# tum-vision/scenedino

Hardware: AMD Instinct MI355X
Metric: rendered rays/sec, KITTI-360 192x640x64-sample frustum (higher is better)
Workload: dtype bf16

## Files before the change

### include/sdhip.h

```cpp
#ifndef SDHIP_H
#define SDHIP_H

#include <stdint.h>

#define SD_CAM_WORDS 36
#include <stddef.h>

#ifdef __cplusplus
extern "C" {
#endif

enum sd_dtype { SD_F32 = 0, SD_BF16 = 1, SD_F16 = 2 };

const char *sd_last_error(void);

int sd_abi_version(void);

int sd_field_dtype(int dtype);

int32_t sd_reserve_cus(int32_t n);

int sd_spin(int32_t nblocks, float us, void *stream);

int sd_gen_rays(const float *poses_c2w, const float *Ks, const float *frame_ids,
// ... 81 lines not shown
    int64_t ld_depth, ld_dino, ld_rgb;
    int32_t grid_dtype;
    int32_t pad1;
} sd_render_args;

int sd_render_fused(const sd_render_args *args, const sd_mlp *mlp, void *stream);


int sd_project_grid(const float *grid_nchw, int64_t B, int64_t Hf, int64_t Wf,
                    const sd_mlp *mlp, void *out, void *stream);

int sd_project_grid_nhwc(const float *grid_nhwc, int64_t B, int64_t Hf, int64_t Wf,
                         const sd_mlp *mlp, void *out, void *stream);

int sd_project_grid_nhwc_inputs(const float *grid_nhwc, int64_t B, int64_t Hf, int64_t Wf,
                                const sd_mlp *mlp, void *out, const sd_frame_args *frame,
                                void *stream);

typedef struct sd_head {
    const void *w_pe;
    const void *w_sig;
    const void *w_out;
    const float *b_dino;
    float b_sigma;
    int32_t D;
    int32_t dtype;
} sd_head;

int sd_render_proj(const sd_render_args *args, const sd_head *head, void *stream);

int64_t sd_render_proj_work_bytes(int64_t R, int32_t D);

int32_t sd_render_tile_cap(int32_t bytes);

typedef struct sd_field_args {
    const float *xyz; int64_t B; int64_t P;
    const void *grid; int32_t Hf, Wf;
    const float *cam_f;
    const float *img; int32_t nv, Hc, Wc;
    const float *cam_c;
    float *sigma;
    float *dino;
    float *rgb;
    float *invalid;
    uint8_t *invalid_f;
    int32_t dino_dtype;
    int32_t grid_dtype;
    const int32_t *tile_order;
} sd_field_args;

int sd_field_query(const sd_field_args *args, const sd_mlp *mlp, void *stream);

int sd_composite(const float *z, const float *sigma, const float *feat, int64_t F,
                 const float *rgb, int64_t Cc, int64_t R, int32_t K, int32_t hard_alpha_cap,
                 float *weights, float *alphas, float *depth, float *feat_out, float *rgb_out,
                 void *stream);


int sd_field_gather(const float *xyz, int64_t B, int64_t P, const float *grid_nhwc,
                    int32_t C, int32_t Hf, int32_t Wf, const float *cam_f,
                    const float *img, int32_t nv, int32_t Hc, int32_t Wc,
                    const float *cam_c, void *x_out, int32_t x_dtype ,
                    uint8_t *invalid_f, float *rgb, float *invalid, void *stream);

int sd_field_gather_bwd(const float *xyz, int64_t B, int64_t P, const void *dx,
                        int32_t dx_dtype , int64_t ldx, int32_t C, int32_t Hf,
// ... 304 lines not shown
```

### scenedino_amd/_lib.py

```python
from __future__ import annotations

import ctypes
import os

import torch

_HERE = os.path.dirname(os.path.abspath(__file__))
LIB_PATH = os.environ.get("SDHIP_LIB") or os.path.join(_HERE, "libsdhip.so")
ABI_VERSION = 12
CAM_WORDS = 36

SD_F32 = 0
SD_BF16 = 1
SD_F16 = 2
TORCH_DTYPE = {SD_F32: torch.float32, SD_BF16: torch.bfloat16, SD_F16: torch.float16}
SD_OF_TORCH = {v: k for k, v in TORCH_DTYPE.items()}
FIELD_DTYPE = {SD_F32: SD_F32, SD_BF16: SD_F16, SD_F16: SD_F16}

_vp = ctypes.c_void_p
_i64 = ctypes.c_int64
_i32 = ctypes.c_int32


class SdMlp(ctypes.Structure):
# ... 170 lines not shown
 SD_EPI_NCHW) = range(8)

SIGNATURES = {
    "sd_last_error": [],
    "sd_abi_version": [],
    "sd_field_dtype": [ctypes.c_int],
    "sd_reserve_cus": [ctypes.c_int32],
    "sd_spin": [ctypes.c_int32, ctypes.c_float, _vp],
    "sd_ln_gemm": [ctypes.POINTER(SdGemmArgs), _vp, _vp, _vp, ctypes.c_float, _vp],
    "sd_gen_rays": [_vp, _vp, _vp, _i64, _i64, _i64, ctypes.c_float, ctypes.c_float, _vp, _vp],
    "sd_sample_z": [_vp, _i64, _i64, _i64, ctypes.c_int, _vp, ctypes.c_uint64, ctypes.c_uint64,
                    _vp, _vp],
    "sd_patch_rays": [ctypes.POINTER(SdPatchArgs), _vp],
    "sd_pack_grid": [_vp, _i64, _i64, _i64, _i64, ctypes.c_int, _vp, _vp],
    "sd_pack_image": [_vp, _i64, _i64, _i64, _vp, _vp],
    "sd_cam_records": [_vp, _i64, _vp, _i64, _i64, _vp, _vp],
    "sd_frame_inputs": [_vp, _i64, _i64, _i64, _vp, _vp, _i64, _vp, _i64, _i64, _vp, _vp],
    "sd_render_fused": [ctypes.POINTER(SdRenderArgs), ctypes.POINTER(SdMlp), _vp],
    "sd_field_query": [ctypes.POINTER(SdFieldArgs), ctypes.POINTER(SdMlp), _vp],
    "sd_field_gather": [_vp, _i64, _i64, _vp, _i32, _i32, _i32, _vp, _vp, _i32, _i32, _i32, _vp,
                        _vp, _i32, _vp, _vp, _vp, _vp],
    "sd_field_gather_bwd": [_vp, _i64, _i64, _vp, _i32, _i64, _i32, _i32, _i32, _vp, _vp, _vp],
    "sd_unpack_grid": [_vp, _i64, _i64, _i64, _i64, _vp, _vp],
    "sd_composite_bwd": [_vp, _vp, _vp, _i64, _vp, _i64, _i64, _i32, _i32, _vp, _vp, _vp, _vp,
                         _vp, _vp, _vp, _vp, _vp],
    "sd_project_grid": [_vp, _i64, _i64, _i64, ctypes.POINTER(SdMlp), _vp, _vp],
    "sd_project_grid_nhwc": [_vp, _i64, _i64, _i64, ctypes.POINTER(SdMlp), _vp, _vp],
    "sd_project_grid_nhwc_inputs": [_vp, _i64, _i64, _i64, ctypes.POINTER(SdMlp), _vp,
                                    ctypes.POINTER(SdFrameArgs), _vp],
    "sd_cast_grid": [_vp, _i64, ctypes.c_int, _vp, _vp],
    "sd_render_proj": [ctypes.POINTER(SdRenderArgs), ctypes.POINTER(SdHead), _vp],
    "sd_render_proj_work_bytes": [_i64, _i32],
    "sd_render_tile_cap": [_i32],
    "sd_composite": [_vp, _vp, _vp, _i64, _vp, _i64, _i64, _i32, _i32, _vp, _vp, _vp, _vp, _vp,
                     _vp],
    "sd_voxel_points": [ctypes.POINTER(ctypes.c_double), ctypes.c_double, _i64, _i64, _i64,
                        ctypes.POINTER(ctypes.c_double), _vp, _vp],
    "sd_grow3": [_vp, _i64, _i64, _i64, _vp, _vp],
    "sd_seg_query": [_vp, _i32, _i64, ctypes.POINTER(SdSegHead), _vp, ctypes.c_float, _vp, _vp,
                     _vp, _vp],
    "sd_voxel_fov": [ctypes.POINTER(ctypes.c_double), ctypes.c_double, _i64, _i64, _i64,
                     ctypes.POINTER(ctypes.c_double), ctypes.POINTER(ctypes.c_double), _i32, _i32,
                     _vp, _vp],
    "sd_ssc_confusion": [_vp, _vp, _vp, _vp, _i64, _i64, _i64, ctypes.POINTER(SdSscArgs), _vp,
                         _vp],
    "sd_mlp_train_fwd": [ctypes.POINTER(SdMlpTrainArgs), _vp],
    "sd_mlp_train_bwd": [ctypes.POINTER(SdMlpTrainArgs), _vp],
    "sd_wgrad": [ctypes.POINTER(SdWgradArgs), _vp],
    "sd_mlp_train_wgrad": [ctypes.POINTER(SdMlpWgradArgs), _vp],
    "sd_mlp_train_wgrad_work": [_i32],
    "sd_salience_fwd": [ctypes.POINTER(SdSalienceArgs), _vp],
    "sd_salience_bwd": [ctypes.POINTER(SdSalienceArgs), _vp],
    "sd_gemm": [ctypes.POINTER(SdGemmArgs), _vp],
    "sd_gemm_resid_ln": [ctypes.POINTER(SdGemmArgs), _vp, _vp, ctypes.c_float, _vp, _vp, _vp],
    "sd_attention": [_vp, _vp, _vp, _i32, _i32, _i32, _i32, _i32, ctypes.c_float, _vp, _vp],
    "sd_vit_mlp": [_vp, _vp, _i64, _i32, _i32, _vp, _vp, ctypes.c_float, _vp, _vp, _vp, _vp, _vp,
                   _vp],
    "sd_layernorm": [_vp, _i64, _i32, _vp, _vp, ctypes.c_float, _vp, _i32, _vp],
    "sd_patchify": [_vp, _i32, _i32, _i32, _i32, _i32, ctypes.POINTER(ctypes.c_float),
                    ctypes.POINTER(ctypes.c_float), _vp, _vp, _vp, _vp, _i32, _vp],
    "sd_tokens_to_grid": [_vp, _i32, _i32, _i32, _i32, _i32, _i32, _i32, _vp, _vp],
    "sd_tokens_to_nhwc": [_vp, _i32, _i32, _i32, _i32, _i32, _i32, _vp, _vp],
    "sd_layernorm_nhwc": [_vp, _i32, _i32, _i32, _vp, _vp, ctypes.c_float, _i32, _i32, _i32, _vp, _vp],
    "sd_upsample2x": [_vp, _i32, _i32, _i32, _i32, _vp, _vp],
    "sd_conv_wgrad_parts": [ctypes.POINTER(SdConvWgradArgs)],
    "sd_conv_wgrad_work": [ctypes.POINTER(SdConvWgradArgs)],
# ... 259 lines not shown
                               ptr(out), stream_of(out)), "sd_project_grid")
    return out


def project_grid_inputs(grid, mlp: SdMlp, dtype, img_nchw, poses_w2c, Ks, exact_grid: bool = False):
    if not channels_last(grid):
        img, cam = frame_inputs(img_nchw, poses_w2c, Ks)
        return project_grid(grid, mlp, dtype, exact_grid), img, cam
    lib = load()
    mlp = _with_flags(mlp, exact_grid)
    B, C, H, W = grid.shape
    N, c3, Hc, Wc = img_nchw.shape
    assert c3 == 3, "colour images must have 3 channels"
    w, k, n, sw, sk = _cam_operands(poses_w2c, Ks)
    out = torch.empty(B, H, W, 128, device=grid.device, dtype=TORCH_DTYPE[FIELD_DTYPE[dtype]])
    img = torch.empty(N, Hc, Wc, 4, device=img_nchw.device, dtype=torch.float32)
    cam = torch.empty(*poses_w2c.shape[:-2], CAM_WORDS, device=w.device, dtype=torch.float32)
    fa = SdFrameArgs(img_nchw=ptr(_req(img_nchw, "images")), N=N, H=Hc, W=Wc, out_nhwc4=ptr(img),
                     w2c=ptr(w), s_w=sw, Ks=ptr(k), s_k=sk, n=n, out_cam=ptr(cam))
    _check(lib.sd_project_grid_nhwc_inputs(ptr(_req(grid.permute(0, 2, 3, 1), "grid")), B, H, W,
                                           ctypes.byref(mlp), ptr(out), ctypes.byref(fa),
                                           stream_of(out)), "sd_project_grid_nhwc_inputs")
    return out, img, cam


def render_proj_work_bytes(R: int, D: int) -> int:
    return int(load().sd_render_proj_work_bytes(R, D))


def render_tile_cap(nbytes: int) -> int:
    return int(load().sd_render_tile_cap(int(nbytes)))


def render_proj(args: SdRenderArgs, head: SdHead, ref_tensor):
    lib = load()
    _check(lib.sd_render_proj(ctypes.byref(args), ctypes.byref(head), stream_of(ref_tensor)),
           "sd_render_proj")


def field_query(args: SdFieldArgs, mlp: SdMlp, ref_tensor):
    lib = load()
    _check(lib.sd_field_query(ctypes.byref(args), ctypes.byref(mlp), stream_of(ref_tensor)),
           "sd_field_query")


def voxel_fov(origin, voxel_size, dims, T, cam_k, img_w, img_h, device):
    lib = load()
    nx, ny, nz = (int(d) for d in dims)
    o = (ctypes.c_double * 3)(*[float(v) for v in origin])
    Tm = torch.as_tensor(T, dtype=torch.float64).reshape(-1, 4)[:3].flatten().tolist()
    t = (ctypes.c_double * 12)(*Tm)
    km = (ctypes.c_double * 9)(*torch.as_tensor(cam_k, dtype=torch.float64)
                               .reshape(3, 3).flatten().tolist())
    out = torch.empty(nx * ny * nz, device=device, dtype=torch.uint8)
    _check(lib.sd_voxel_fov(o, float(voxel_size), nx, ny, nz, t, km, int(img_w), int(img_h),
                            ptr(out), stream_of(out)), "sd_voxel_fov")
    return out


def ssc_confusion(pred, sigma, target, fov, args: SdSscArgs, conf):
    lib = load()
    nx, ny, nz = (int(d) for d in pred.shape)
    _check(lib.sd_ssc_confusion(ptr(pred), ptr(sigma), ptr(target), ptr(fov), nx, ny, nz,
                                ctypes.byref(args), ptr(conf), stream_of(conf)),
           "sd_ssc_confusion")

# ... 538 lines not shown
```

### scenedino_amd/csrc/sdhip_tile.hip

```cpp
#include "sdhip_render.h"
#include <stdlib.h>

#ifndef ST_NW_SMALLK
#define ST_NW_SMALLK 8
#endif
#define ST_TEX 288
#define ST_TEXQ 18
#define ST_MAXP 2
#define ST_MAXKW 8

#ifndef ST_PROF
#define ST_PROF 0
#endif
#if ST_PROF
__device__ unsigned long long st_prof[32];
#define ST_T(i)                                                  \
    {                                                            \
        const uint64_t _t = __builtin_amdgcn_s_memtime();        \
        pacc[i] += (uint32_t)(_t - tlast);                       \
        tlast = _t;                                              \
    }
extern "C" int sd_tile_prof(unsigned long long *out, int reset) {
    if (hipMemcpyFromSymbol(out, HIP_SYMBOL(st_prof), sizeof(st_prof)) != hipSuccess) return -2;
    if (reset) {
        unsigned long long z[32] = {0};
        if (hipMemcpyToSymbol(HIP_SYMBOL(st_prof), z, sizeof(z)) != hipSuccess) return -2;
    }
    return 0;
}
#elif defined(ST_MARK) && ST_MARK
#define ST_T(i) asm volatile(";@T " #i)
#else
#define ST_T(i)
#endif
#ifndef ST_MARK
#define ST_MARK 0
#endif
#if ST_MARK
#define ST_M(i) asm volatile(";@M " #i)
#define ST_MV(i, x) asm volatile(";@M " #i : "+v"(x))
#else
// ... 12 lines not shown
#endif
#ifndef ST_SAME_CAM
#define ST_SAME_CAM 1
#endif
#ifndef ST_FASTPROJ
#define ST_FASTPROJ 1
#endif
#if ST_FASTPROJ
#define ST_GEO sd_point_geo_fast
#define ST_CTAPS sd_color_taps_fast
#else
#define ST_GEO sd_point_geo<true>
#define ST_CTAPS sd_color_taps
#endif

struct st_args {
    sd_render_args a;
    sd_head m;
    int32_t *ovf;
    int32_t ovf_cap;
    int32_t ngroups;
    int32_t tile_bytes;
};

#define ST_L_BOX 0
#define ST_HS_ROW 272
__host__ __device__ constexpr int st_l_hs(int nw) { return ST_L_BOX + 2 * nw * 32; }
__host__ __device__ constexpr int st_l_ws(int nw, int rpw) { return st_l_hs(nw) + nw * rpw * ST_HS_ROW; }
__host__ __device__ constexpr int st_l_ray(int nw, int rpw) { return st_l_ws(nw, rpw) + 16 * 4; }
__host__ __device__ constexpr int st_l_rec(int nw, int rpw) { return st_l_ray(nw, rpw) + nw * 2 * 32 * rpw; }
static_assert(st_l_rec(8, 1) % 16 == 0 && st_l_rec(12, 1) % 16 == 0 && st_l_rec(8, 2) % 16 == 0,
              "record area alignment");

__host__ __device__ constexpr int st_rec_bytes(int nw, int kw) { return nw * 2 * kw * 40; }

#define ST_BFLY(NOP, out, a, b, RA, RB, MA, MB)                                               \
    asm volatile(NOP "v_add_f32_dpp %0, %1, %1 row_ror:" #RA " row_mask:0xf bank_mask:" #MA "\n\t" \
                 "v_add_f32_dpp %0, %2, %2 row_ror:" #RB " row_mask:0xf bank_mask:" #MB      \
                 : "=&v"(out) : "v"(a), "v"(b))

__device__ __forceinline__ uint32_t st_min2(uint32_t a, uint32_t b) {
    typedef __attribute__((ext_vector_type(2))) unsigned short u16x2;
    return __builtin_bit_cast(uint32_t, __builtin_elementwise_min(__builtin_bit_cast(u16x2, a),
                                                                  __builtin_bit_cast(u16x2, b)));
}
__device__ __forceinline__ uint32_t st_max2(uint32_t a, uint32_t b) {
    typedef __attribute__((ext_vector_type(2))) unsigned short u16x2;
    return __builtin_bit_cast(uint32_t, __builtin_elementwise_max(__builtin_bit_cast(u16x2, a),
                                                                  __builtin_bit_cast(u16x2, b)));
}
template <bool MAX>
__device__ __forceinline__ uint32_t st_row_red2(uint32_t v) {
#define ST_RSTEP(ctrl)                                                                        \
    {                                                                                         \
        const uint32_t o = (uint32_t)__builtin_amdgcn_mov_dpp((int)v, (ctrl), 0xf, 0xf, false); \
        v = MAX ? st_max2(v, o) : st_min2(v, o);                                              \
    }
    ST_RSTEP(0xB1)
    ST_RSTEP(0x4E)
    ST_RSTEP(0x141)
    ST_RSTEP(0x140)
#undef ST_RSTEP
    return v;
}
template <bool MAX>
__device__ __forceinline__ uint32_t st_rows2(uint32_t v, int r0, int r1) {
    uint32_t acc = (uint32_t)__builtin_amdgcn_readlane((int)v, 16 * r0);
// ... 27 lines not shown
#define ST_EARLY_HW ST_WAIT_EARLY
#endif
#ifndef ST_PRIO
#define ST_PRIO 0
#endif
#ifndef ST_EARLY_FETCH
#define ST_EARLY_FETCH 1
#endif
typedef unsigned u32x4v __attribute__((ext_vector_type(4)));
__device__ __forceinline__ void st_out(float *p, float v) {
    if (ST_WT)
        __hip_atomic_store(p, v, __ATOMIC_RELAXED, __HIP_MEMORY_SCOPE_AGENT);
    else
        *p = v;
}

__device__ __forceinline__ void st_dma4(const void *src, uint32_t lds_addr) {
    lds_addr = __builtin_amdgcn_readfirstlane(lds_addr);
    asm volatile("s_mov_b32 m0, %1\n\ts_nop 0\n\tglobal_load_lds_dword %0, off"
                 :: "v"(src), "s"(lds_addr) : "memory");
}
__device__ __forceinline__ void st_dma_buf16(__amdgpu_buffer_rsrc_t rs, uint32_t voff, uint32_t soff,
                                             uint32_t lds_addr) {
    asm volatile("s_mov_b32 m0, %2\n\ts_nop 0\n\tbuffer_load_dwordx4 %0, %1, %3 offen lds"
                 :: "v"(voff), "s"(rs), "s"(lds_addr), "s"(soff) : "memory");
}
typedef __attribute__((ext_vector_type(4))) short s16x4;

__device__ __forceinline__ uint2 st_tr(uint32_t addr) {
    const s16x4 v = __builtin_amdgcn_ds_read_tr16_b64_v4i16((__attribute__((address_space(3))) s16x4 *)(uintptr_t)addr);
    return __builtin_bit_cast(uint2, v);
}

template <int P, bool ZIN, int NW, int RPW>
__global__ void __launch_bounds__(64 * NW) __attribute__((amdgpu_waves_per_eu(NW / 4)))
k_render_tile(const st_args sa) {
#ifndef ST_HPRE_RPW2
#define ST_HPRE_RPW2 2
#endif
    constexpr int HPRE = (RPW == 2 && ST_HEAD_PRE == 3) ? ST_HPRE_RPW2 : ST_HEAD_PRE;
    constexpr int ST_WAVES = NW;
    constexpr int GR = NW * RPW;
    constexpr int ST_L_HS = st_l_hs(NW), ST_L_WS = st_l_ws(NW, RPW), ST_L_RAY = st_l_ray(NW, RPW),
                  ST_L_REC = st_l_rec(NW, RPW);
    typedef typename RMode<P>::F Tr;
    typedef typename RMode<P>::H Th;
    typedef typename Tr::Frag Frag;
    typedef typename Tr::Frag4 Frag4;
    typedef typename Tr::E E;
    const sd_render_args &a = sa.a;
    const sd_head &m = sa.m;
    extern __shared__ __attribute__((aligned(16))) uint8_t lds[];
#if ST_PROF
    uint32_t pacc[19] = {};
    uint64_t tlast = __builtin_amdgcn_s_memtime();
#endif
    const uint32_t lds0 = (uint32_t)(uintptr_t)(lds_void *)lds;

    const int lane = threadIdx.x & 63, j = lane & 15, g = lane >> 4;
    const int wave = __builtin_amdgcn_readfirstlane(threadIdx.x >> 6);
    const int K = a.K, nsub = K >> 4;
    const int KW = K * RPW, nsubw = KW >> 4;
    const int R = (int)a.R, rps = (int)a.rays_per_sb;
    const int D = m.D, ndt = D >> 4;
    const int Wf = a.Wf, Hf = a.Hf;
    const uint32_t plane_bytes = (uint32_t)Hf * Wf * SD_DH * 2;

    const uint32_t rec_base = ST_L_REC + (uint32_t)wave * 2 * KW * 40;
    auto rq0 = [&](int buf) { return (uint4 *)(lds + rec_base + buf * KW * 40); };
    auto rq1 = [&](int buf) { return (f32x4 *)(lds + rec_base + buf * KW * 40 + KW * 16); };
    auto rqc = [&](int buf) { return (float2 *)(lds + rec_base + buf * KW * 40 + KW * 32); };
    const uint32_t tile0 = ST_L_REC + st_rec_bytes(NW, KW);

    const int NG = sa.ngroups;
    const int nx = (gridDim.x % 8 == 0) ? 8 : 1;
    const int xcd = blockIdx.x % nx, lb = blockIdx.x / nx, nwg = gridDim.x / nx;
    const int glo = (int)((int64_t)NG * xcd / nx), ghi = (int)((int64_t)NG * (xcd + 1) / nx);
    const int gfirst = glo + lb;
    const int nsteps = gfirst < ghi ? (ghi - gfirst + nwg - 1) / nwg : 0;
    int novf = 0;
    int32_t *ovf_list = sa.ovf + gridDim.x + (int64_t)blockIdx.x * sa.ovf_cap;
    if (nsteps == 0) {
        if (threadIdx.x == 0) sa.ovf[blockIdx.x] = 0;
        return;
    }

    const float zstep = (float)(1.0 / (double)K), zend = (float)(1.0 - 1.0 / (double)K);
    const int64_t cplane = (int64_t)a.Hc * a.Wc * 4;

    const int nrw = min(a.ray_dim, 8);
    auto rmap = [&](int ray_, int r) { return RPW == 1 ? ray_ + r : ray_ - RPW * wave + r * NW + wave; };
    auto ray_fetch = [&](int ray, int slot) {
        const int r = lane >> 3, w = lane & 7;
        if (r < RPW && w < nrw && rmap(ray, r) < R)
            st_dma4(a.rays + (int64_t)rmap(ray, r) * a.ray_dim + w,
                    lds0 + ST_L_RAY + (wave * 2 + slot) * 32 * RPW);
    };
    const int rsl = RPW == 1 ? 0 : min(lane / K, RPW - 1);
    auto rsl_p = [&](int p) { return RPW == 1 ? 0 : min((64 * p + lane) / K, RPW - 1); };
    auto kl_p = [&](int p) { return RPW == 1 ? 64 * p + lane : 64 * p + lane - rsl_p(p) * K; };
    const float *rl = nullptr;
    auto load_ray_z = [&](int ray, float zq[2 * ST_MAXP]) {
        float zo[ST_MAXP];
        if (ZIN) {
            if (RPW == 1) {
// ... 116 lines not shown
            q[1] = st_rows2<true>(mx0, 0, 1);
            q[2] = st_rows2<false>(mn0, 2, 3);
            q[3] = st_rows2<true>(mx0, 2, 3);
            q[4] = st_rows2<false>(mn1, 0, 1);
            q[5] = st_rows2<true>(mx1, 0, 1);
            q[6] = st_rows2<false>(mn1, 2, 3);
            q[7] = st_rows2<true>(mx1, 2, 3);
            ST_T(12);
            if (lane == 0) {
                *(uint4 *)bw = uint4{q[0], q[1], q[2], q[3]};
                *(uint4 *)(bw + 16) = uint4{q[4], q[5], q[6], q[7]};
            }
        } else {
            bmin0 = st_wave_min2(bmin0);
            bmax0 = st_wave_max2(bmax0);
            bmin1 = st_wave_min2(bmin1);
            bmax1 = st_wave_max2(bmax1);
            ST_T(12);
            if (lane == 0) *(uint4 *)bw = uint4{bmin0, bmax0, bmin1, bmax1};
        }
    };
    auto ray_col = [&](int ray, int buf) {
        if (rmap(ray, rsl) < R && lane < KW) {
            float col[3];
            sd_color_finish(cpend, col);
            rq0(buf)[lane].w = __builtin_bit_cast(uint32_t, col[0]);
            rqc(buf)[lane] = float2{col[1], col[2]};
        }
    };

    struct Tile {
        int bx0, by0, tw, th, pitch, ok, split;
    };
    const int NPART = (KW == 64 || (RPW == 2 && KW == 128)) ? 4 : 2;
    auto box_union = [&](int slot, int p0, int p1, uint32_t &mn, uint32_t &mx) {
        const uint4 *bx = (const uint4 *)(lds + ST_L_BOX + slot * ST_WAVES * 32);
        mn = 0xffffffffu;
        mx = 0u;
        if (lane < 2 * ST_WAVES) {
            const uint4 v = bx[lane];
            const int pa = 2 * (lane & 1);
            if (pa >= p0 && pa < p1) {
                mn = v.x;
                mx = v.y;
            }
            if (pa + 1 >= p0 && pa + 1 < p1) {
                mn = st_min2(mn, v.z);
                mx = st_max2(mx, v.w);
            }
        }
        static_assert(2 * ST_WAVES <= 16, "box entries in lane row 0");
        mn = st_rows2<false>(st_row_red2<false>(mn), 0, 0);
        mx = st_rows2<true>(st_row_red2<true>(mx), 0, 0);
    };
    auto geom = [&](uint32_t mn, uint32_t mx) {
        Tile t;
        t.bx0 = (int)(mn & 0xffffu);
        t.by0 = (int)(mn >> 16);
        t.tw = (int)(mx & 0xffffu) - t.bx0 + 1;
        t.th = (int)(mx >> 16) - t.by0 + 1;
        t.pitch = t.tw > 0 ? st_pitch(t.tw) : 1;
        t.ok = (mn != 0xffffffffu) && t.tw > 0 && t.th > 0 &&
               t.th * t.pitch * ST_TEX <= sa.tile_bytes && (t.tw * ST_TEXQ + 63) / 64 <= ST_MAXKW * ST_WAVES;
        t.split = 0;
        return t;
    };
    auto dma = [&](const Tile &t, int tb, int sbi) {
// ... 71 lines not shown
            gp[p] = t.pitch;
        }
        const int np = t.split + 1;
#pragma unroll 1
        for (int q = 1; q < np; ++q) {
            uint32_t mn1, mx1;
            box_union(rbuf, q * NPART / np, (q + 1) * NPART / np, mn1, mx1);
            const Tile tq = geom(mn1, mx1);
            const int s0 = q * nsubw / np, s1 = (q + 1) * nsubw / np;
#pragma unroll
            for (int p = 0; p < ST_MAXP; ++p) {
                const int it = (64 * p + lane) >> 4;
                const bool mine = it >= s0 && it < s1;
                gx[p] = mine ? tq.bx0 : gx[p];
                gy[p] = mine ? tq.by0 : gy[p];
                gp[p] = mine ? tq.pitch : gp[p];
            }
        }
        const uint32_t tbase = lds0 + tile0 + (uint32_t)tb * (uint32_t)sa.tile_bytes;
        uint32_t *w = (uint32_t *)rq0(rbuf);
#pragma unroll
        for (int p = 0; p < ST_MAXP; ++p) {
            const int k = 64 * p + lane;
            if (64 * p < KW && k < KW) {
                const uint32_t xy = w[4 * k];
                const int bx0 = gx[p], by0 = gy[p], pch = gp[p];
                const int x0 = (int)(xy & 0x7fffu), y0 = (int)((xy >> 15) & 0x7fffu);
                const uint32_t ad = tbase + (uint32_t)(((y0 - by0) * pch + (x0 - bx0)) * ST_TEX);
                w[4 * k] = ad | (xy & 0xc0000000u);
            }
        }
    };

    typedef typename Th::Frag HFrag;
#ifndef ST_BD_HOIST1
#define ST_BD_HOIST1 0
#endif
    constexpr bool BDH = RPW == 2 || ST_BD_HOIST1;
    f32x4 bdw = {0.f, 0.f, 0.f, 0.f};
    if (BDH && wave < ndt) bdw = *(const f32x4 *)(m.b_dino + 16 * wave + 4 * g);
    auto head_w = [&](int dt, HFrag w[4]) {
        const HFrag *wo = (const HFrag *)m.w_out + (int64_t)dt * 4 * SD_WAVE + lane;
#pragma unroll
        for (int s = 0; s < 4; ++s) w[s] = wo[s * SD_WAVE];
    };
    auto head = [&](int grp, const HFrag w0[4]) {
        if (wave >= ndt) return;
        const int slot = j < GR ? j : 0;
        typename Th::Frag Bh[4];
        const uint8_t *hs = lds + ST_L_HS + slot * ST_HS_ROW;
#pragma unroll
        for (int s = 0; s < 4; ++s) {
            const uint2 lo = *(const uint2 *)(hs + (32 * s + 4 * g) * 2);
            const uint2 hi = *(const uint2 *)(hs + (32 * s + 16 + 4 * g) * 2);
            Bh[s] = __builtin_bit_cast(typename Th::Frag, uint4{lo.x, lo.y, hi.x, hi.y});
        }
        const float ws = *(const float *)(lds + ST_L_WS + slot * 4);
        const int ray = GR * grp + (RPW == 1 ? j : (j % RPW) * NW + j / RPW);
        const bool store = j < GR && ray < R;
        for (int dt = wave; dt < ndt; dt += ST_WAVES) {
            HFrag wl[4];
            if ((HPRE == 1 || HPRE == 3) && dt == wave) {
#pragma unroll
                for (int s = 0; s < 4; ++s) wl[s] = w0[s];
            } else {
                head_w(dt, wl);
// ... 15 lines not shown
                        (uint32_t)(((int64_t)(ray - GR * grp) * a.ld_dino + dim) * 4), 0, 16);
                } else {
                    *(f32x4 *)(a.dino + (int64_t)ray * a.ld_dino + dim) = res;
                }
            }
        }
    };

    const int tq = (lane & 15) >> 2, tp = lane & 3;
    const bool bsel = ((j & 7) >> 1) == g;
    const bool bc0 = bsel && (j >> 3) == 0, bc1 = bsel && (j >> 3) == 1;
    const bool br1 = (j & 1) != 0;
    const f32x4 zero4 = {0.f, 0.f, 0.f, 0.f};
    Frag wpe[8];
    Frag4 wpe1[8];
#pragma unroll
    for (int t = 0; t < 8; ++t) {
        wpe[t] = ((const Frag *)m.w_pe)[t * SD_WAVE + lane];
        wpe1[t] = ((const Frag4 *)((const uint8_t *)m.w_pe + 8 * SD_WAVE * 16))[t * SD_WAVE + lane];
    }
    uint4 wsig_r[4];
#pragma unroll
    for (int s2 = 0; s2 < 4; ++s2) wsig_r[s2] = ((const uint4 *)m.w_sig)[s2 * SD_WAVE + lane];
#if ST_WAIT_FIX
    __builtin_amdgcn_s_waitcnt(0x0F70);
#endif

    int grp = gfirst;
    int ray = GR * grp + RPW * wave;
    int sbi = __builtin_amdgcn_readfirstlane((int)((unsigned)min(GR * grp, R - 1) / (unsigned)rps));
    ray_fetch(ray, 0);
    ray_fetch(GR * (grp + nwg) + RPW * wave, 1);
    asm volatile("s_waitcnt vmcnt(0)" ::: "memory");
    ray_pass(ray, 0, 0);
    ray_col(ray, 0);
    st_barrier_lds();
    Tile cur = stage(0, 0, grp, sbi);
    tap_addrs(0, 0, cur, ray);
    asm volatile("s_waitcnt vmcnt(0)" ::: "memory");
    __syncthreads();

    if (ST_PRIO == 1 && wave >= NW / 2) __builtin_amdgcn_s_setprio(1);
    if (ST_PRIO == 2 && wave < NW / 2) __builtin_amdgcn_s_setprio(1);
    int prev_grp = -1, prev_ok = 0;
    HFrag hwn[4];
#if ST_PROF
#pragma unroll
    for (int i = 0; i < 19; ++i) pacc[i] = 0;
    tlast = __builtin_amdgcn_s_memtime();
#endif
    for (int n = 0; n < nsteps; ++n) {
        const int buf = n & 1;
        const bool has_next = n + 1 < nsteps;
        const int ngrp = grp + nwg;
        const int nray = GR * ngrp + RPW * wave;
        const int nsbi = has_next ? __builtin_amdgcn_readfirstlane((int)((unsigned)min(GR * ngrp, R - 1) / (unsigned)rps)) : 0;
        uint32_t lane_off = (uint32_t)((tq & 1) + (tq >> 1) * cur.pitch) * ST_TEX + 8u * (uint32_t)tp;

        float Tc, dpart, wpart, cpart[3];
#if ST_HC16
        f16x2 hacc16[16];
#else
        f32x4 hacc[8];
#endif
        auto reset = [&]() {
            Tc = 1.f;
            dpart = wpart = cpart[0] = cpart[1] = cpart[2] = 0.f;
#if ST_HC16
#pragma unroll
            for (int i = 0; i < 16; ++i) hacc16[i] = f16x2{(_Float16)0.f, (_Float16)0.f};
#else
#pragma unroll
            for (int t = 0; t < 8; ++t) hacc[t] = zero4;
// ... 85 lines not shown
            cpart[1] += w * st.col[1];
            cpart[2] += w * st.col[2];
            ST_MV(27, cpart[2]);
#if ST_HC16
            const f16x2 ww = __builtin_bit_cast(f16x2, sd_pack2<_Float16>(w, w));
#pragma unroll
            for (int s2 = 0; s2 < 4; ++s2) {
                const uint4 u = __builtin_bit_cast(uint4, st.X[s2]);
                const uint32_t d4[4] = {u.x, u.y, u.z, u.w};
#pragma unroll
                for (int q = 0; q < 4; ++q)
                    hacc16[4 * s2 + q] = __builtin_elementwise_fma(__builtin_bit_cast(f16x2, d4[q]), ww,
                                                                   hacc16[4 * s2 + q]);
            }
#else
            const uint32_t wl = sd_pack2<E>(w, 0.f), wh = sd_pack2<E>(0.f, w);
#pragma unroll
            for (int s2 = 0; s2 < 4; ++s2) {
                const uint4 u = __builtin_bit_cast(uint4, st.X[s2]);
                const uint32_t d4[4] = {u.x, u.y, u.z, u.w};
#pragma unroll
                for (int q = 0; q < 4; ++q) {
                    const int t = 2 * s2 + (q >> 1), r = 2 * (q & 1);
                    hacc[t][r] = Tr::dot2(d4[q], wl, hacc[t][r]);
                    hacc[t][r + 1] = Tr::dot2(d4[q], wh, hacc[t][r + 1]);
                }
            }
#endif
            if (g == 0) *(float2 *)&rq1(buf)[k] = float2{w, st.alpha};
            ST_M(28);
        };

        HFrag hw[4];
        if (HPRE == 1 && prev_ok && wave < ndt) head_w(wave, hw);
        if (HPRE == 2 && prev_ok) head(prev_grp, hw);
        if (HPRE == 3 && prev_ok) head(prev_grp, hwn);
        if (HPRE >= 2) ST_T(1);
        if (has_next) ray_pass(nray, buf ^ 1, buf ^ 1);
        ST_T(0);
        if (HPRE < 2 && prev_ok) head(prev_grp, hw);
        if (HPRE < 2) ST_T(1);
        IState s0;
        if (cur.ok && ray < R) itemA(0, s0);
        ST_T(2);
        if (has_next) ray_col(nray, buf ^ 1);
        ST_T(3);
        st_barrier_lds();
        ST_T(4);
        Tile nxt = {0, 0, 0, 0, 1, 0, 0};
        if (has_next) {
            nxt = stage(buf ^ 1, buf ^ 1, ngrp, nsbi);
            tap_addrs(buf ^ 1, buf ^ 1, nxt, nray);
        }
        if (ST_EARLY_FETCH && n + 2 < nsteps) ray_fetch(GR * (ngrp + nwg) + RPW * wave, buf);
        if (ST_EARLY_HW && HPRE == 3 && cur.ok && wave < ndt) head_w(wave, hwn);
        ST_T(5);
        const int npart = cur.split + 1;
        int qn = 1, bnd = npart > 1 ? nsubw / npart : nsubw;
        auto ray_sums = [&](int r) {
            const float dsum = sd_rowsum16(dpart), wsum = sd_rowsum16(wpart);
            const float c0s = sd_rowsum16(cpart[0]), c1s = sd_rowsum16(cpart[1]),
                        c2s = sd_rowsum16(cpart[2]);
            uint8_t *hs = lds + ST_L_HS + (wave * RPW + r) * ST_HS_ROW;
            {
#if ST_HC16
                float hacc[8][4];
#pragma unroll
                for (int s2 = 0; s2 < 4; ++s2)
#pragma unroll
                    for (int q = 0; q < 4; ++q) {
                        const int t = 2 * s2 + (q >> 1), r = 2 * (q & 1);
                        const uint32_t hb = __builtin_bit_cast(uint32_t, hacc16[4 * s2 + q]);
                        hacc[t][r] = (float)__builtin_bit_cast(_Float16, (uint16_t)(hb & 0xffffu));
                        hacc[t][r + 1] = (float)__builtin_bit_cast(_Float16, (uint16_t)(hb >> 16));
                    }
#endif
                float u[16], v[8];
                asm volatile("s_nop 1" : "+v"(hacc[0][0]), "+v"(hacc[0][1]), "+v"(hacc[0][2]), "+v"(hacc[0][3]),
                             "+v"(hacc[1][0]), "+v"(hacc[1][1]), "+v"(hacc[1][2]), "+v"(hacc[1][3]),
                             "+v"(hacc[2][0]), "+v"(hacc[2][1]), "+v"(hacc[2][2]), "+v"(hacc[2][3]),
                             "+v"(hacc[3][0]), "+v"(hacc[3][1]), "+v"(hacc[3][2]), "+v"(hacc[3][3]));
                asm volatile("s_nop 1" : "+v"(hacc[4][0]), "+v"(hacc[4][1]), "+v"(hacc[4][2]), "+v"(hacc[4][3]),
                             "+v"(hacc[5][0]), "+v"(hacc[5][1]), "+v"(hacc[5][2]), "+v"(hacc[5][3]),
                             "+v"(hacc[6][0]), "+v"(hacc[6][1]), "+v"(hacc[6][2]), "+v"(hacc[6][3]),
                             "+v"(hacc[7][0]), "+v"(hacc[7][1]), "+v"(hacc[7][2]), "+v"(hacc[7][3]));
// ... 48 lines not shown
                if (act) ray_sums(r);
                reset();
            }
        }
        if (ST_WAIT_EARLY) asm volatile("s_waitcnt vmcnt(0)" ::: "memory");
        ST_T(6);
        if (cur.ok && rmap(ray, RPW - 1) < R) ray_sums(RPW - 1);
        if (cur.ok) {
#pragma unroll
            for (int p = 0; p < ST_MAXP; ++p) {
                const int kr = 64 * p + lane;
                const int rr = RPW == 1 ? 0 : min(kr / K, RPW - 1);
                const int k = kr - rr * K;
                if (64 * p < KW && kr < KW && rmap(ray, rr) < R) {
                    const int64_t rk = (int64_t)rmap(ray, rr) * K;
                    const f32x4 q1v = rq1(buf)[kr];
                    const uint4 q0v = rq0(buf)[kr];
                    const uint32_t fl = q0v.x >> 30;
                    if (a.weights) st_out(a.weights + rk + k, q1v[0]);
                    if (a.alphas) st_out(a.alphas + rk + k, q1v[1]);
                    if (a.invalid_f) a.invalid_f[rk + k] = (uint8_t)(fl & 1u);
                    if (a.invalid) st_out(a.invalid + rk + k, fl ? 1.f : 0.f);
                    if (a.rgb_samps) {
                        const float2 cgb = rqc(buf)[kr];
                        float *rsp = a.rgb_samps + (rk + k) * 3;
                        st_out(rsp, __builtin_bit_cast(float, q0v.w));
                        st_out(rsp + 1, cgb.x);
                        st_out(rsp + 2, cgb.y);
                    }
                }
            }
        }
        ST_T(7);
        prev_grp = grp;
        prev_ok = cur.ok;
        grp = ngrp;
        ray = nray;
        sbi = nsbi;
        cur = nxt;
        if (!ST_EARLY_FETCH && n + 2 < nsteps) ray_fetch(GR * (ngrp + nwg) + RPW * wave, buf);
        if (!ST_EARLY_HW && HPRE == 3 && prev_ok && wave < ndt) head_w(wave, hwn);
        if (!ST_WAIT_EARLY) asm volatile("s_waitcnt vmcnt(0)" ::: "memory");
        ST_T(8);
        st_barrier_lds();
        ST_T(9);
    }
    if (threadIdx.x == 0) sa.ovf[blockIdx.x] = novf;
    if (prev_ok) {
        if (HPRE == 1) {
            HFrag hw[4];
            if (wave < ndt) head_w(wave, hw);
            head(prev_grp, hw);
        } else {
            head(prev_grp, hwn);
        }
    }
#if ST_PROF
    if (lane < 19) {
        uint32_t v = 0;
#pragma unroll
        for (int i = 0; i < 19; ++i) v = lane == i ? pacc[i] : v;
        atomicAdd(&st_prof[lane], (unsigned long long)v);
    }
    if (lane == 0) atomicAdd(&st_prof[31], 1ull);
#endif
}

static int sd_check_last(const char *what) {
    hipError_t e = hipGetLastError();
    if (e != hipSuccess) {
        sd_set_error(hipGetErrorString(e));
        (void)what;
        return -2;
    }
    return 0;
}

static int st_nw(int K) { return K <= 64 ? ST_NW_SMALLK : 8; }

static int st_rpw(int K) {
    static const int force = getenv("SDHIP_TILE_RPW") ? atoi(getenv("SDHIP_TILE_RPW")) : 0;
    const int kmax = force == 2 ? 64 : 32;
    return (K <= kmax && force != 1 && st_nw(K) == 8) ? 2 : 1;
}

static int st_lds_fixed(int K) {
    const int nw = st_nw(K), rpw = st_rpw(K);
    return st_l_rec(nw, rpw) + st_rec_bytes(nw, K * rpw);
}

static int st_cap_bytes = 0;
extern "C" int32_t sd_render_tile_cap(int32_t bytes) {
    const int prev = st_cap_bytes;
    st_cap_bytes = bytes > 0 ? bytes : 0;
    return prev;
}

static int st_tile_bytes(int K) {
    const int avail = 160 * 1024 - st_lds_fixed(K);
    const int b = ((avail / 2) / 1024) * 1024;
    return st_cap_bytes ? min(b, (st_cap_bytes / 1024) * 1024) : b;
}

extern "C" int sd_render_tile_ok(const sd_render_args *a, const sd_head *m) {
    return a->nv == 1 && a->K % 16 == 0 && a->K <= 128 &&
           a->rays_per_sb % (st_nw(a->K) * st_rpw(a->K)) == 0 &&
           m->D % 16 == 0 && m->D <= 512 && a->Wf < 32768 && a->Hf < 32768 &&
           st_tile_bytes(a->K) >= 16 * 1024;
}

extern "C" int sd_render_tile_launch(const sd_render_args *a, const sd_head *m, int32_t *ovf,
                                     void *stream) {
    hipStream_t s = (hipStream_t)stream;
    st_args sa;
    sa.a = *a;
    sa.m = *m;
    sa.ovf = ovf;
    const int ncu = sd_num_cus();
    sa.ovf_cap = (int32_t)sd_ovf_cap(a->R, ncu);
    const int nw = st_nw(a->K), rpw = st_rpw(a->K);
    sa.ngroups = (int)((a->R + nw * rpw - 1) / (nw * rpw));
    sa.tile_bytes = st_tile_bytes(a->K);
    const int lds_bytes = st_lds_fixed(a->K) + 2 * sa.tile_bytes;
    auto go = [&](auto kern) {
        sd_lds_attr((const void *)kern, lds_bytes);
        hipLaunchKernelGGL(kern, dim3((unsigned)ncu), dim3(64 * nw), lds_bytes, s, sa);
    };
    const bool zin = a->z != nullptr;
#define ST_GO(NWV, RPWV)                                                                              \
    if (m->dtype == SD_F16) {                                                                         \
        if (zin) go(k_render_tile<SD_F16, true, NWV, RPWV>); else go(k_render_tile<SD_F16, false, NWV, RPWV>); \
    } else {                                                                                          \
        if (zin) go(k_render_tile<SD_BF16, true, NWV, RPWV>); else go(k_render_tile<SD_BF16, false, NWV, RPWV>); \
    }
    if (nw == 8 && rpw == 2) {
        ST_GO(8, 2)
    } else if (nw == 8) {
        ST_GO(8, 1)
    } else {
        ST_GO(ST_NW_SMALLK, 1)
    }
#undef ST_GO
    return sd_check_last("sd_render_proj (tile kernel)");
}
```

Measured before the change: 211.7 million.

## Add late-order tile schedule: box pass first, per-sample geometry after staging

Adds a LATE variant of the tile render kernel. It first computes only a conservative bounding box from a few sample points per ray, stages the feature tile, and then recomputes the full per-sample geometry, tap records and colour after the tile loads are issued, overlapping that work with the loads. Rays whose samples fall outside the predicted box are flagged through LDS and sent to the overflow list. This halves the record buffering in LDS, which leaves room for larger tiles. It is the default for K=64 with RPW=2 and accepts non-divisible rays_per_sb when there is a single superbatch. The trade-off is duplicated geometry work, a coarse box estimate that can send more groups to the overflow path, and a changed meaning for the SDHIP_TILE_RPW env var.

```diff
diff --git a/include/sdhip.h b/include/sdhip.h
--- a/include/sdhip.h
+++ b/include/sdhip.h
@@ -137,6 +137,8 @@
 int64_t sd_render_proj_work_bytes(int64_t R, int32_t D);
 
 int32_t sd_render_tile_cap(int32_t bytes);
+
+int32_t sd_render_tile_order(int32_t order);
 
 typedef struct sd_field_args {
     const float *xyz; int64_t B; int64_t P;
diff --git a/scenedino_amd/_lib.py b/scenedino_amd/_lib.py
--- a/scenedino_amd/_lib.py
+++ b/scenedino_amd/_lib.py
@@ -226,6 +226,7 @@
     "sd_render_proj": [ctypes.POINTER(SdRenderArgs), ctypes.POINTER(SdHead), _vp],
     "sd_render_proj_work_bytes": [_i64, _i32],
     "sd_render_tile_cap": [_i32],
+    "sd_render_tile_order": [_i32],
     "sd_composite": [_vp, _vp, _vp, _i64, _vp, _i64, _i64, _i32, _i32, _vp, _vp, _vp, _vp, _vp,
                      _vp],
     "sd_voxel_points": [ctypes.POINTER(ctypes.c_double), ctypes.c_double, _i64, _i64, _i64,
@@ -551,6 +552,10 @@
     return int(load().sd_render_tile_cap(int(nbytes)))
 
 
+def render_tile_order(order: int) -> int:
+    return int(load().sd_render_tile_order(int(order)))
+
+
 def render_proj(args: SdRenderArgs, head: SdHead, ref_tensor):
     lib = load()
     _check(lib.sd_render_proj(ctypes.byref(args), ctypes.byref(head), stream_of(ref_tensor)),
diff --git a/scenedino_amd/csrc/sdhip_tile.hip b/scenedino_amd/csrc/sdhip_tile.hip
--- a/scenedino_amd/csrc/sdhip_tile.hip
+++ b/scenedino_amd/csrc/sdhip_tile.hip
@@ -7,6 +7,7 @@
 #define ST_TEX 288
 #define ST_TEXQ 18
 #define ST_MAXP 2
+#define ST_BOX_EPS (1.f / 1024.f)
 #define ST_MAXKW 8
 
 #ifndef ST_PROF
@@ -85,7 +86,9 @@
 static_assert(st_l_rec(8, 1) % 16 == 0 && st_l_rec(12, 1) % 16 == 0 && st_l_rec(8, 2) % 16 == 0,
               "record area alignment");
 
-__host__ __device__ constexpr int st_rec_bytes(int nw, int kw) { return nw * 2 * kw * 40; }
+__host__ __device__ constexpr int st_rec_bytes(int nw, int kw, bool late = false) {
+    return late ? nw * kw * 40 + 16 : nw * 2 * kw * 40;
+}
 
 #define ST_BFLY(NOP, out, a, b, RA, RB, MA, MB)                                               \
     asm volatile(NOP "v_add_f32_dpp %0, %1, %1 row_ror:" #RA " row_mask:0xf bank_mask:" #MA "\n\t" \
@@ -179,7 +182,7 @@
     return __builtin_bit_cast(uint2, v);
 }
 
-template <int P, bool ZIN, int NW, int RPW>
+template <int P, bool ZIN, int NW, int RPW, bool LATE = false>
 __global__ void __launch_bounds__(64 * NW) __attribute__((amdgpu_waves_per_eu(NW / 4)))
 k_render_tile(const st_args sa) {
 #ifndef ST_HPRE_RPW2
@@ -206,18 +209,19 @@
 
     const int lane = threadIdx.x & 63, j = lane & 15, g = lane >> 4;
     const int wave = __builtin_amdgcn_readfirstlane(threadIdx.x >> 6);
-    const int K = a.K, nsub = K >> 4;
+    const int K = LATE ? 128 / RPW : a.K, nsub = K >> 4;
     const int KW = K * RPW, nsubw = KW >> 4;
     const int R = (int)a.R, rps = (int)a.rays_per_sb;
     const int D = m.D, ndt = D >> 4;
     const int Wf = a.Wf, Hf = a.Hf;
     const uint32_t plane_bytes = (uint32_t)Hf * Wf * SD_DH * 2;
 
-    const uint32_t rec_base = ST_L_REC + (uint32_t)wave * 2 * KW * 40;
-    auto rq0 = [&](int buf) { return (uint4 *)(lds + rec_base + buf * KW * 40); };
-    auto rq1 = [&](int buf) { return (f32x4 *)(lds + rec_base + buf * KW * 40 + KW * 16); };
-    auto rqc = [&](int buf) { return (float2 *)(lds + rec_base + buf * KW * 40 + KW * 32); };
-    const uint32_t tile0 = ST_L_REC + st_rec_bytes(NW, KW);
+    const uint32_t rec_base = ST_L_REC + (uint32_t)wave * (LATE ? 1 : 2) * KW * 40;
+    auto rq0 = [&](int buf) { return (uint4 *)(lds + rec_base + (LATE ? 0 : buf) * KW * 40); };
+    auto rq1 = [&](int buf) { return (f32x4 *)(lds + rec_base + (LATE ? 0 : buf) * KW * 40 + KW * 16); };
+    auto rqc = [&](int buf) { return (float2 *)(lds + rec_base + (LATE ? 0 : buf) * KW * 40 + KW * 32); };
+    const uint32_t tile0 = ST_L_REC + st_rec_bytes(NW, KW, LATE);
+    const uint32_t flag0 = tile0 - 16;
 
     const int NG = sa.ngroups;
     const int nx = (gridDim.x % 8 == 0) ? 8 : 1;
@@ -400,7 +404,7 @@
     struct Tile {
         int bx0, by0, tw, th, pitch, ok, split;
     };
-    const int NPART = (KW == 64 || (RPW == 2 && KW == 128)) ? 4 : 2;
+    const int NPART = (LATE || KW == 64 || (RPW == 2 && KW == 128)) ? 4 : 2;
     auto box_union = [&](int slot, int p0, int p1, uint32_t &mn, uint32_t &mx) {
         const uint4 *bx = (const uint4 *)(lds + ST_L_BOX + slot * ST_WAVES * 32);
         mn = 0xffffffffu;
@@ -538,6 +542,136 @@
         }
     };
 
+    auto samp_geo = [&](const float *rw, int rmem, int k, int sbi_, float &z0, float &px, float &py,
+                        float &pz) {
+        if (ZIN)
+            z0 = a.z[(int64_t)rmem * K + k];
+        else
+            z0 = sd_z_sample_rng(rw[6], rw[7], K, k,
+                                 sd_uniform(a.z_seed, a.z_offset + (uint64_t)rmem * (uint64_t)K + k), zstep,
+                                 zend, a.z_lindisp);
+        px = rw[0] + z0 * rw[3];
+        py = rw[1] + z0 * rw[4];
+        pz = rw[2] + z0 * rw[5];
+        return ST_GEO((sd_cfloat *)(a.cam_f + sbi_ * SD_CAM_WORDS), px, py, pz, Wf, Hf);
+    };
+    auto box_pass = [&](int ray_, int slot, int sbi_) {
+        const int e = lane & 7;
+        const int kr = 32 * (e >> 1) + ((e & 1) ? 31 : 0);
+        const int r = RPW == 1 ? 0 : kr / K, k = kr - r * K;
+        const int rmem = rmap(ray_, r);
+        uint32_t mn = 0xffffffffu, mx = 0u;
+        if (rmem < R) {
+            const float *rw = (const float *)(lds + ST_L_RAY + (wave * 2 + slot) * 32 * RPW) + 8 * r;
+            float z0, px, py, pz;
+            const PointGeo geo = samp_geo(rw, rmem, k, sbi_, z0, px, py, pz);
+            const float fx = geo.t.w01 + geo.t.w11, fy = geo.t.w10 + geo.t.w11;
+            const int xl = max(geo.t.x0 - (fx < ST_BOX_EPS ? 1 : 0), 0);
+            const int yl = max(geo.t.y0 - (fy < ST_BOX_EPS ? 1 : 0), 0);
+            const int xh = min(geo.t.x0 + (fx > 1.f - ST_BOX_EPS ? 1 : 0), Wf - 1);
+            const int yh = min(geo.t.y0 + (fy > 1.f - ST_BOX_EPS ? 1 : 0), Hf - 1);
+            mn = (uint32_t)xl | ((uint32_t)yl << 16);
+            mx = ((uint32_t)xh | ((uint32_t)yh << 16)) + 0x00010001u;
+        }
+        mn = st_min2(mn, (uint32_t)__builtin_amdgcn_mov_dpp((int)mn, 0xB1, 0xf, 0xf, false));
+        mx = st_max2(mx, (uint32_t)__builtin_amdgcn_mov_dpp((int)mx, 0xB1, 0xf, 0xf, false));
+        uint32_t q[8];
+#pragma unroll
+        for (int i = 0; i < 4; ++i) {
+            q[2 * i] = (uint32_t)__builtin_amdgcn_readlane((int)mn, 2 * i);
+            q[2 * i + 1] = (uint32_t)__builtin_amdgcn_readlane((int)mx, 2 * i);
+        }
+        if (lane == 0) {
+            uint8_t *bw = lds + ST_L_BOX + (slot * ST_WAVES + wave) * 32;
+            *(uint4 *)bw = uint4{q[0], q[1], q[2], q[3]};
+            *(uint4 *)(bw + 16) = uint4{q[4], q[5], q[6], q[7]};
+        }
+    };
+    auto late_pass = [&](int ray_, int slot, int tb, const Tile &t, int sbi_) {
+        if (!t.ok) return;
+        int gx[ST_MAXP], gy[ST_MAXP], gp[ST_MAXP], gw[ST_MAXP], gh[ST_MAXP];
+#pragma unroll
+        for (int p = 0; p < ST_MAXP; ++p) {
+            gx[p] = t.bx0;
+            gy[p] = t.by0;
+            gp[p] = t.pitch;
+            gw[p] = t.tw;
+            gh[p] = t.th;
+        }
+        const int np = t.split + 1;
+#pragma unroll 1
+        for (int q = 1; q < np; ++q) {
+            uint32_t mn1, mx1;
+            box_union(slot, q * NPART / np, (q + 1) * NPART / np, mn1, mx1);
+            const Tile tq = geom(mn1, mx1);
+            const int s0 = q * nsubw / np, s1 = (q + 1) * nsubw / np;
+#pragma unroll
+            for (int p = 0; p < ST_MAXP; ++p) {
+                const int it = (64 * p + lane) >> 4;
+                const bool mine = it >= s0 && it < s1;
+                gx[p] = mine ? tq.bx0 : gx[p];
+                gy[p] = mine ? tq.by0 : gy[p];
+                gp[p] = mine ? tq.pitch : gp[p];
+                gw[p] = mine ? tq.tw : gw[p];
+                gh[p] = mine ? tq.th : gh[p];
+            }
+        }
+        const uint32_t tbase = lds0 + tile0 + (uint32_t)tb * (uint32_t)sa.tile_bytes;
+        const float *rl_ = (const float *)(lds + ST_L_RAY + (wave * 2 + slot) * 32 * RPW);
+        const bool same_cam = ST_SAME_CAM && a.cam_c == a.cam_f && a.Wc == Wf && a.Hc == Hf;
+        uint4 *r0 = rq0(0);
+        f32x4 *r1 = rq1(0);
+        float2 *rc = rqc(0);
+        bool miss = false;
+#pragma unroll
+        for (int p = 0; p < ST_MAXP; ++p) {
+            const int kr = 64 * p + lane;
+            const int r = RPW == 1 ? 0 : kr / K, k = kr - r * K;
+            const int rmem = rmap(ray_, r);
+            if (rmem < R) {
+                float z0, px, py, pz;
+                const PointGeo geo = samp_geo(rl_ + 8 * r, rmem, k, sbi_, z0, px, py, pz);
+                bool ic;
+                Taps tc;
+                if (same_cam) {
+                    tc = geo.t;
+                    ic = geo.inv_f;
+                } else {
+                    tc = ST_CTAPS((sd_cfloat *)(a.cam_c + sbi_ * SD_CAM_WORDS), a.Wc, a.Hc, px, py, pz, ic);
+                }
+                const int dx = geo.t.x0 - gx[p], dy = geo.t.y0 - gy[p];
+                miss |= (uint32_t)dx >= (uint32_t)(gw[p] - 1) || (uint32_t)dy >= (uint32_t)(gh[p] - 1);
+                const uint32_t ad = tbase + (uint32_t)((dy * gp[p] + dx) * ST_TEX);
+                const uint32_t xy = (ad & 0x3fffffffu) | (geo.inv_f ? 1u << 30 : 0u) | (ic ? 1u << 31 : 0u);
+                const uint4 wp = sd_pack_w<SD_F16>(geo.t.w00, geo.t.w01, geo.t.w10, geo.t.w11);
+                r1[kr] = f32x4{geo.v[0], geo.v[1], geo.v[2], z0};
+                if (p == 0) {
+                    sd_color_issue(a.img + (int64_t)sbi_ * cplane, tc, cpend);
+                    r0[kr] = uint4{xy, wp.x, wp.y, 0u};
+                } else {
+                    float col[3];
+                    sd_sample_rgb(a.img + (int64_t)sbi_ * cplane, tc, col);
+                    r0[kr] = uint4{xy, wp.x, wp.y, __builtin_bit_cast(uint32_t, col[0])};
+                    rc[kr] = float2{col[1], col[2]};
+                }
+            }
+        }
+        if (__builtin_amdgcn_ballot_w64(miss) != 0ull && lane == 0)
+            *(volatile uint32_t *)(lds + flag0 + 4 * slot) = 1u;
+    };
+    auto late_check = [&](int slot, Tile &t, int g_) {
+        if (!t.ok) return;
+        const uint32_t f = (uint32_t)__builtin_amdgcn_readfirstlane(
+            (int)*(volatile uint32_t *)(lds + flag0 + 4 * slot));
+        if (!f) return;
+        t.ok = 0;
+        if (wave == 0 && lane == 0) {
+            for (int b = 0; b < GR / SD_LIST_BLK; ++b)
+                ovf_list[novf + b] = g_ * (GR / SD_LIST_BLK) + b;
+        }
+        novf += GR / SD_LIST_BLK;
+    };
+
     typedef typename Th::Frag HFrag;
 #ifndef ST_BD_HOIST1
 #define ST_BD_HOIST1 0
@@ -619,13 +753,26 @@
     ray_fetch(ray, 0);
     ray_fetch(GR * (grp + nwg) + RPW * wave, 1);
     asm volatile("s_waitcnt vmcnt(0)" ::: "memory");
-    ray_pass(ray, 0, 0);
-    ray_col(ray, 0);
-    st_barrier_lds();
-    Tile cur = stage(0, 0, grp, sbi);
-    tap_addrs(0, 0, cur, ray);
-    asm volatile("s_waitcnt vmcnt(0)" ::: "memory");
-    __syncthreads();
+    Tile cur;
+    if constexpr (LATE) {
+        static_assert(HPRE >= 2, "late order: the head runs in front of the box pass");
+        if (threadIdx.x == 0) *(uint2 *)(lds + flag0) = uint2{0u, 0u};
+        box_pass(ray, 0, sbi);
+        st_barrier_lds();
+        cur = stage(0, 0, grp, sbi);
+        late_pass(ray, 0, 0, cur, sbi);
+        asm volatile("s_waitcnt vmcnt(0)" ::: "memory");
+        __syncthreads();
+        late_check(0, cur, grp);
+    } else {
+        ray_pass(ray, 0, 0);
+        ray_col(ray, 0);
+        st_barrier_lds();
+        cur = stage(0, 0, grp, sbi);
+        tap_addrs(0, 0, cur, ray);
+        asm volatile("s_waitcnt vmcnt(0)" ::: "memory");
+        __syncthreads();
+    }
 
     if (ST_PRIO == 1 && wave >= NW / 2) __builtin_amdgcn_s_setprio(1);
     if (ST_PRIO == 2 && wave < NW / 2) __builtin_amdgcn_s_setprio(1);
@@ -777,25 +924,38 @@
         };
 
         HFrag hw[4];
-        if (HPRE == 1 && prev_ok && wave < ndt) head_w(wave, hw);
-        if (HPRE == 2 && prev_ok) head(prev_grp, hw);
-        if (HPRE == 3 && prev_ok) head(prev_grp, hwn);
-        if (HPRE >= 2) ST_T(1);
-        if (has_next) ray_pass(nray, buf ^ 1, buf ^ 1);
-        ST_T(0);
-        if (HPRE < 2 && prev_ok) head(prev_grp, hw);
-        if (HPRE < 2) ST_T(1);
         IState s0;
-        if (cur.ok && ray < R) itemA(0, s0);
-        ST_T(2);
-        if (has_next) ray_col(nray, buf ^ 1);
-        ST_T(3);
+        if constexpr (LATE) {
+            if (HPRE == 2 && prev_ok) head(prev_grp, hw);
+            if (HPRE == 3 && prev_ok) head(prev_grp, hwn);
+            ST_T(1);
+            if (has_next) box_pass(nray, buf ^ 1, nsbi);
+            ST_T(12);
+            if (cur.ok) ray_col(ray, buf);
+            ST_T(3);
+            if (cur.ok && rmap(ray, 0) < R) itemA(0, s0);
+            ST_T(2);
+        } else {
+            if (HPRE == 1 && prev_ok && wave < ndt) head_w(wave, hw);
+            if (HPRE == 2 && prev_ok) head(prev_grp, hw);
+            if (HPRE == 3 && prev_ok) head(prev_grp, hwn);
+            if (HPRE >= 2) ST_T(1);
+            if (has_next) ray_pass(nray, buf ^ 1, buf ^ 1);
+            ST_T(0);
+            if (HPRE < 2 && prev_ok) head(prev_grp, hw);
+            if (HPRE < 2) ST_T(1);
+            if (cur.ok && ray < R) itemA(0, s0);
+            ST_T(2);
+            if (has_next) ray_col(nray, buf ^ 1);
+            ST_T(3);
+        }
         st_barrier_lds();
         ST_T(4);
+        if (LATE && threadIdx.x == 0) *(volatile uint32_t *)(lds + flag0 + 4 * buf) = 0u;
         Tile nxt = {0, 0, 0, 0, 1, 0, 0};
         if (has_next) {
             nxt = stage(buf ^ 1, buf ^ 1, ngrp, nsbi);
-            tap_addrs(buf ^ 1, buf ^ 1, nxt, nray);
+            if (!LATE) tap_addrs(buf ^ 1, buf ^ 1, nxt, nray);
         }
         if (ST_EARLY_FETCH && n + 2 < nsteps) ray_fetch(GR * (ngrp + nwg) + RPW * wave, buf);
         if (ST_EARLY_HW && HPRE == 3 && cur.ok && wave < ndt) head_w(wave, hwn);
@@ -910,6 +1070,10 @@
             }
         }
         ST_T(7);
+        if constexpr (LATE) {
+            if (has_next) late_pass(nray, buf ^ 1, buf ^ 1, nxt, nsbi);
+            ST_T(0);
+        }
         prev_grp = grp;
         prev_ok = cur.ok;
         grp = ngrp;
@@ -922,6 +1086,7 @@
         ST_T(8);
         st_barrier_lds();
         ST_T(9);
+        if constexpr (LATE) late_check(buf ^ 1, cur, grp);
     }
     if (threadIdx.x == 0) sa.ovf[blockIdx.x] = novf;
     if (prev_ok) {
@@ -956,15 +1121,32 @@
 
 static int st_nw(int K) { return K <= 64 ? ST_NW_SMALLK : 8; }
 
+static int st_order_init() {
+    const char *e = getenv("SDHIP_TILE_RPW");
+    const int v = e ? atoi(e) : 0;
+    return v >= 0 && v <= 4 ? v : 0;
+}
+static int st_order_v = st_order_init();
+extern "C" int32_t sd_render_tile_order(int32_t order) {
+    const int prev = st_order_v;
+    if (order >= 0 && order <= 4) st_order_v = order;
+    return prev;
+}
+
+static bool st_late(int K) {
+    if (st_nw(K) != 8) return false;
+    return st_order_v == 3 ? (K == 64 || K == 128) : st_order_v == 0 && K == 64;
+}
+
 static int st_rpw(int K) {
-    static const int force = getenv("SDHIP_TILE_RPW") ? atoi(getenv("SDHIP_TILE_RPW")) : 0;
-    const int kmax = force == 2 ? 64 : 32;
-    return (K <= kmax && force != 1 && st_nw(K) == 8) ? 2 : 1;
+    if (st_nw(K) != 8 || st_order_v == 1) return 1;
+    if (st_late(K)) return K == 64 ? 2 : 1;
+    return K <= (st_order_v == 2 ? 64 : 32) ? 2 : 1;
 }
 
 static int st_lds_fixed(int K) {
     const int nw = st_nw(K), rpw = st_rpw(K);
-    return st_l_rec(nw, rpw) + st_rec_bytes(nw, K * rpw);
+    return st_l_rec(nw, rpw) + st_rec_bytes(nw, K * rpw, st_late(K));
 }
 
 static int st_cap_bytes = 0;
@@ -982,7 +1164,8 @@
 
 extern "C" int sd_render_tile_ok(const sd_render_args *a, const sd_head *m) {
     return a->nv == 1 && a->K % 16 == 0 && a->K <= 128 &&
-           a->rays_per_sb % (st_nw(a->K) * st_rpw(a->K)) == 0 &&
+           (a->rays_per_sb % (st_nw(a->K) * st_rpw(a->K)) == 0 ||
+            (st_late(a->K) && a->R == a->rays_per_sb)) &&
            m->D % 16 == 0 && m->D <= 512 && a->Wf < 32768 && a->Hf < 32768 &&
            st_tile_bytes(a->K) >= 16 * 1024;
 }
@@ -1005,18 +1188,24 @@
         hipLaunchKernelGGL(kern, dim3((unsigned)ncu), dim3(64 * nw), lds_bytes, s, sa);
     };
     const bool zin = a->z != nullptr;
-#define ST_GO(NWV, RPWV)                                                                              \
+#define ST_GO(NWV, RPWV, LATEV)                                                                       \
     if (m->dtype == SD_F16) {                                                                         \
-        if (zin) go(k_render_tile<SD_F16, true, NWV, RPWV>); else go(k_render_tile<SD_F16, false, NWV, RPWV>); \
+        if (zin) go(k_render_tile<SD_F16, true, NWV, RPWV, LATEV>);                                   \
+        else go(k_render_tile<SD_F16, false, NWV, RPWV, LATEV>);                                      \
     } else {                                                                                          \
-        if (zin) go(k_render_tile<SD_BF16, true, NWV, RPWV>); else go(k_render_tile<SD_BF16, false, NWV, RPWV>); \
+        if (zin) go(k_render_tile<SD_BF16, true, NWV, RPWV, LATEV>);                                  \
+        else go(k_render_tile<SD_BF16, false, NWV, RPWV, LATEV>);                                     \
     }
-    if (nw == 8 && rpw == 2) {
-        ST_GO(8, 2)
+    if (st_late(a->K) && rpw == 2) {
+        ST_GO(8, 2, true)
+    } else if (st_late(a->K)) {
+        ST_GO(8, 1, true)
+    } else if (nw == 8 && rpw == 2) {
+        ST_GO(8, 2, false)
     } else if (nw == 8) {
-        ST_GO(8, 1)
+        ST_GO(8, 1, false)
     } else {
-        ST_GO(ST_NW_SMALLK, 1)
+        ST_GO(ST_NW_SMALLK, 1, false)
     }
 #undef ST_GO
     return sd_check_last("sd_render_proj (tile kernel)");
```

Measured after the change: 235.4 million, median of 6. +11.2%, better.
